# Martinsos/edlib

Hardware: AMD Instinct MI355X
Metric: GCUPS (cell updates/s), 1M x 150bp HW reads vs 5Mb target (higher is better)
Workload: dtype u32

## Files before the change

edlib_amd/csrc/engine.hip:

```cpp
#include "engine.hpp"
#include "flat_results.hpp"
#include <sched.h>

#if defined(__x86_64__)
#include <immintrin.h>
#endif
#include <algorithm>
#include <chrono>
#include <atomic>
#include <cmath>
#include <cstdarg>
#include <cstring>
#include <condition_variable>
#include <mutex>
#include <system_error>
#include <thread>

namespace edlib_amd {


static void build_eq8(std::vector<uint8_t>& eq8, const EdlibEqualityPair* eqs, int neq) {
    eq8.assign(256 * 256, 0);
    for (int a = 0; a < 256; ++a) eq8[a * 256 + a] = 1;
    for (int i = 0; i < neq; ++i) {
// ... 61 lines not shown
            if (tab.eq8.empty() ? (q == tab.idToByte[s]) : (tab.eq8[q * 256 + tab.idToByte[s]] != 0)) mask |= (uint16_t)(1u << s);
        tab.eqtbl[q] = mask;
    }
}


__global__ void __launch_bounds__(256)
alphabet_count_kernel(const uint8_t* __restrict__ qpool, const long long* __restrict__ qoff,
                      const uint8_t* __restrict__ tpool, const long long* __restrict__ toff,
                      int shared, const uint32_t* __restrict__ basePresence,
                      const int* __restrict__ unitIdx, int* __restrict__ out)
{
    __shared__ uint32_t s_seen[256];
    s_seen[threadIdx.x] = 0u;
    __syncthreads();
    const int u = unitIdx[blockIdx.x];
    auto scan = [&](const uint8_t* pool, long long lo, long long hi) {
        for (long long c = (lo >> 4) + threadIdx.x; (c << 4) < hi; c += 256) {
            const uint4 v = *reinterpret_cast<const uint4*>(pool + (c << 4));
            const uint32_t d[4] = {v.x, v.y, v.z, v.w};
            const long long at = c << 4;
            if (at >= lo && at + 16 <= hi) {
#pragma unroll
                for (int k = 0; k < 16; ++k) s_seen[(d[k >> 2] >> (8 * (k & 3))) & 0xffu] = 1u;
            } else {
#pragma unroll
                for (int k = 0; k < 16; ++k)
                    if (at + k >= lo && at + k < hi) s_seen[(d[k >> 2] >> (8 * (k & 3))) & 0xffu] = 1u;
            }
        }
    };
    scan(qpool, qoff[u], qoff[u + 1]);
    if (!shared) scan(tpool, toff[u], toff[u + 1]);
    __syncthreads();
    bool present = s_seen[threadIdx.x] != 0u;
    if (shared) present = present || ((basePresence[threadIdx.x >> 5] >> (threadIdx.x & 31)) & 1u);
    const int n = __syncthreads_count(present ? 1 : 0);
    if (threadIdx.x == 0) out[blockIdx.x] = n;
}

__global__ void __launch_bounds__(256)
alphabet_count_short_kernel(const uint8_t* __restrict__ qpool, const long long* __restrict__ qoff,
                            const uint8_t* __restrict__ tpool, const long long* __restrict__ toff,
                            int shared, const uint32_t* __restrict__ basePresence,
                            const int* __restrict__ unitIdx, int n, int* __restrict__ out)
{
    __shared__ uint32_t s_seen[4][64];
    const int lane = threadIdx.x & 63, wv = threadIdx.x >> 6;
    const int slot = blockIdx.x * 4 + wv;
    if (slot >= n) return;
    uint8_t* const seen = reinterpret_cast<uint8_t*>(s_seen[wv]);
    s_seen[wv][lane] = 0u;
    const int u = unitIdx[slot];
    auto scan = [&](const uint8_t* pool, long long lo, long long hi) {
        for (long long c = (lo >> 4) + lane; (c << 4) < hi; c += 64) {
            const uint4 v = *reinterpret_cast<const uint4*>(pool + (c << 4));
            const uint32_t d[4] = {v.x, v.y, v.z, v.w};
            const long long at = c << 4;
#pragma unroll
            for (int k = 0; k < 16; ++k)
                if (at + k >= lo && at + k < hi) seen[(d[k >> 2] >> (8 * (k & 3))) & 0xffu] = 1;
        }
    };
    scan(qpool, qoff[u], qoff[u + 1]);
    if (!shared) scan(tpool, toff[u], toff[u + 1]);
    __builtin_amdgcn_fence(__ATOMIC_RELEASE, "wavefront");
    __builtin_amdgcn_wave_barrier();
    uint32_t w = s_seen[wv][lane];
    if (shared) {
        const uint32_t bits = (basePresence[lane >> 3] >> (4 * (lane & 7))) & 0xfu;
        w |= (bits & 1u) | ((bits & 2u) << 7) | ((bits & 4u) << 14) | ((bits & 8u) << 21);
    }
    int cnt = ((w & 0xffu) != 0) + ((w & 0xff00u) != 0) + ((w & 0xff0000u) != 0) + ((w & 0xff000000u) != 0);
#pragma unroll
    for (int off = 32; off >= 1; off >>= 1) cnt += __shfl_xor(cnt, off, 64);
    if (lane == 0) out[slot] = cnt;
}


Batch::~Batch() {
    DeviceGuard guard(device_);
    if (side_) { (void)hipStreamSynchronize(side_); pool_stream_release(side_); }
    if (aux_) { (void)hipStreamSynchronize(aux_); (void)hipStreamDestroy(aux_); }
    if (stream_) { (void)hipStreamSynchronize(stream_); pool_stream_release(stream_); }
    wideGateRelease();
    for (auto& p : scanEvents_) { pool_event_release(p.first, device_); pool_event_release(p.second, device_); }
}

int roundup(int x, int q) { return (x + q - 1) / q * q; }

int Batch::init(const char* queries, const long long* qoff, int n, const char* targets,
                const long long* toff, int numTargets, EdlibAlignConfig cfg, int device, bool bothStrands, bool hits)
{
    if (n < 0 || (numTargets != 1 && numTargets != n)) { set_error("bad batch shape"); return 1; }
    if (hits) {
        if (numTargets != 1 || bothStrands) { set_error("hit-list read batch: one shared target, one strand"); return 1; }
        if (cfg.mode != EDLIB_MODE_HW) { set_error("hit-list read batch: config.mode must be EDLIB_MODE_HW (SHW and NW have no hit list)"); return 1; }
        if (cfg.task != EDLIB_TASK_DISTANCE) {
            set_error("hit-list read batch: config.task must be EDLIB_TASK_DISTANCE (start locations and paths: align the chosen windows with a pair batch)");
            return 1;
        }
        if (cfg.k < 0) { set_error("hit-list read batch: config.k must be >= 0 (got %d)", cfg.k); return 1; }
        for (int u = 0; u < n; ++u)
            if (qoff[u + 1] - qoff[u] > 32LL * kMaxReadWords) {
                set_error("hit-list read batch: read %d has %lld bases, the limit is %d", u, qoff[u + 1] - qoff[u], 32 * kMaxReadWords);
                return 1;
            }
        bool seen[256] = {false};
        int sigma = 0;
        for (long long j = toff[0]; j < toff[1]; ++j) if (!seen[(uint8_t)targets[j]]) { seen[(uint8_t)targets[j]] = true; ++sigma; }
        if (sigma > 16) { set_error("hit-list read batch: the target has %d distinct symbols, the limit is 16", sigma); return 1; }
    }
    hits_ = hits;
    if (bothStrands && (numTargets != 1 || n > 0x3fffffff)) { set_error("bad both-strand batch shape"); return 1; }
    if (check_device(device)) return 1;
    keep_config(cfg, cfg_, eqs_);
    device_ = device;
    strands_ = bothStrands;
    shared_ = (numTargets == 1);
    if (copy_offsets(qoff, n, "query", qoff_)) return 1;
    const int numReads = n;
    const long long qb = qoff[0];
    if (strands_) {
        n = 2 * numReads;
        qoff_.resize((size_t)n + 1);
        for (int i = 0; i < numReads; ++i) { qoff_[2 * i] = 2 * (qoff[i] - qb); qoff_[2 * i + 1] = 2 * (qoff[i] - qb) + (qoff[i + 1] - qoff[i]); }
        qoff_[n] = 2 * (qoff[numReads] - qb);
    }
    n_ = n;
    if (copy_offsets(toff, numTargets, "target", toff_)) return 1;
    const long long qbytes = qoff_[n] - qoff_[0], tbytes = toff_[numTargets] - toff_[0];
    build_tables(tab_, reinterpret_cast<const uint8_t*>(targets) + toff_[0], tbytes,
                 eqs_.data(), (int)eqs_.size());

    pool_quarantine(false);
    DeviceGuard guard(device_);
    EDLIB_AMD_HIP(guard.status);
    EDLIB_AMD_HIP(pool_stream(&stream_));
    EDLIB_AMD_HIP(evRun0_.create()); EDLIB_AMD_HIP(evRun1_.create());

    const long long tb = toff_[0];
    if (!strands_) for (auto& v : qoff_) v -= qb;
    for (auto& v : toff_) v -= tb;
    {
        const bool inlineT = qbytes + tbytes <= (1 << 20), inlineQ = inlineT && !strands_;
        size_t at = 0;
        auto take = [&](size_t bytes) { const size_t o = at; at = (at + bytes + 15) & ~(size_t)15; return o; };
        const size_t oQoff = take(qoff_.size() * sizeof(long long)), oToff = take(toff_.size() * sizeof(long long));
        const size_t oTlut = take(256), oId = take(256), oEq4 = take(512), oPres = take(32);
        const size_t oQ = inlineQ ? take((size_t)qbytes + 16) : 0, oT = inlineT ? take((size_t)tbytes + 16) : 0;
        EDLIB_AMD_HIP(d_in_.alloc(at));
        EDLIB_AMD_HIP(h_in_.alloc(at));
        uint8_t* h = h_in_.p;
        memcpy(h + oQoff, qoff_.data(), qoff_.size() * sizeof(long long));
        memcpy(h + oToff, toff_.data(), toff_.size() * sizeof(long long));
        memcpy(h + oTlut, tab_.tlut, 256); memcpy(h + oId, tab_.idToByte, 256);
        memcpy(h + oEq4, tab_.eqtbl, 512); memcpy(h + oPres, tab_.presence, 32);
        d_qoff_.alias(d_in_.p + oQoff, qoff_.size()); d_toff_.alias(d_in_.p + oToff, toff_.size());
        d_tlut_.alias(d_in_.p + oTlut, 256); d_idToByte_.alias(d_in_.p + oId, 256);
        d_eqtbl_.alias(d_in_.p + oEq4, 256); d_presence_.alias(d_in_.p + oPres, 8);
        if (inlineQ) {
            if (qbytes) memcpy(h + oQ, queries + qb, (size_t)qbytes);
            memset(h + oQ + qbytes, 0, 16);
            d_qpool_.alias(d_in_.p + oQ, (size_t)qbytes + 16);
        } else {
            EDLIB_AMD_HIP(d_qpool_.alloc((size_t)qbytes + 16));
// ... 868 lines not shown
```

edlib_amd/csrc/engine.hpp:

```cpp
#pragma once
#include "../../include/edlib_amd.h"
#include "common.hpp"
#include "pair_kernels.hpp"
#include "lanepair.hpp"
#include "reads_kernels.hpp"
#include "cross_kernels.hpp"
#include "window_kernels.hpp"
#include "strands.hpp"

#include <chrono>
#include <deque>
#include <functional>
#include <memory>
#include <vector>

namespace edlib_amd {

struct Tables {
    uint8_t tlut[256];
    uint8_t idToByte[256];
    int sigmaT = 0;
    uint32_t presence[8];
    uint16_t eqtbl[256];
    std::vector<uint8_t> eq8;
// ... 100 lines not shown
    int alphabetLength = 0;
    bool hasEnds = false, hasStarts = false, hasAlignment = false;
    LocList ends, starts;
    const uint8_t* opsView = nullptr;
    int opsViewLen = 0;
};

struct Lap;
struct ViewLayout;

class Batch {
public:
    virtual ~Batch();
    int init(const char* queries, const long long* qoff, int n,
             const char* targets, const long long* toff, int numTargets,
             EdlibAlignConfig cfg, int device, bool bothStrands = false,
             bool hits = false);
    int run();
    int runImpl();
    int results(EdlibAlignResult* out);
    int resultsFlat(int* status, int* editDistance, int* numLocations, int* alphabetLength, long long* locOffsets,
                    int** endLocations, int** startLocations, long long* alnOffsets, unsigned char** alignment);
    int resultsView(EdlibAmdResultsView* out);
    int cigarView(int format, const char** chars, const long long** offsets);
    int strandView(EdlibAmdStrandView* out);
    int hitsView(EdlibAmdReadHits* out);
    bool isHits() const { return hits_; }
    EdlibAmdBatchStats stats{};
    void finishStats();

private:
    EdlibAlignConfig cfg_{};
    std::vector<EdlibEqualityPair> eqs_;
    int device_ = 0;
    bool shared_ = false;
    int n_ = 0;
    std::vector<long long> qoff_, toff_;
    bool strands_ = false;
    PinBuf h_strand_;
    int outN() const { return strands_ ? n_ / 2 : n_; }
    int unitOf(int u) const { return strands_ ? 2 * u + h_strand_.p[u] : u; }
    void setStrand(int read, int code) { h_strand_.p[read] = (uint8_t)(code & kStrandReverse); h_strand_.p[outN() + read] = (code & kStrandBoth) ? 1 : 0; }
    int resolveStrandsOnHost(std::vector<UnitResult>& res);
    int hostStrandCounts_[4] = {0, 0, 0, 0};
    int strandCounts(int counts[4]);
    Tables tab_;
    hipStream_t stream_ = nullptr;
    Event evRun0_, evRun1_, evA_, evB_;

    DevBuf<uint8_t> d_in_;
    PinBuf h_in_;
    DevBuf<uint8_t> d_qpool_, d_tpool_, d_tlut_, d_idToByte_, d_eq8_;
    DevBuf<uint16_t> d_eqtbl_;
    hipError_t uploadEq8();
    DevBuf<uint32_t> d_presence_;
    DevBuf<long long> d_qoff_, d_toff_;

    std::vector<int> emptyUnits_, readUnits_, pairUnits_;
    std::vector<int> longUnits_;
    std::vector<int> pairNow_;
    int beginRun(hipError_t guardStatus);
    int enqueueWordSteps();
    int endRun();
    void resetRecords(std::vector<UnitResult>& res);
    void answerEmptyUnits(std::vector<UnitResult>& res);
    int runFlatPhase(std::vector<UnitResult>& res, Lap& lap);
    int runLongReads(std::vector<UnitResult>& res, Lap& lap);
    int runPairPhase(std::vector<UnitResult>& res, Lap& lap);
    int runStartsPhase(std::vector<UnitResult>& res, Lap& lap);
    int runPathsPhase(std::vector<UnitResult>& res, Lap& lap);
    void startStats();
    bool flatDone_ = false;

    struct ReadGroup {
        int nwords = 0, nslots = 0, numSegments = 1, segLen = 0, warm = 0, mMin = 0;
        std::vector<int> perm;
        DevBuf<int> d_perm, d_qlen, d_kinit, d_alphaExtra, d_segBest, d_segCnt, d_segPos;
        DevBuf<int> d_best, d_total, d_pos, d_flags;
        DevBuf<uint32_t> d_peq;
        bool zeroCopy = false; PinBuf hostOut;
        std::vector<int> ovfSlots; std::vector<long long> ovfOff; DevBuf<int> d_ovfPool;
        DevBuf<int> d_lvMap, d_lvBest, d_lvCnt, d_lvPos; std::vector<int> lvMap; int lvS = 0, lvCap = 0; bool lvValid = false;
        DevBuf<int> d_list;
        int nreal = -1;
        bool mates = false; DevBuf<int> d_win;
    };
    static constexpr int kLastLevelCap = 16;
    int listOpenSlots(ReadGroup& g, int kDone, std::vector<int>& out);
    DevBuf<uint8_t> d_selTmp_;
    std::vector<std::unique_ptr<ReadGroup>> groups_;
    DevBuf<uint32_t> d_tpk_, d_trows_;
    DevBuf<unsigned long long> d_wordSteps_;
    PinBuf h_wordSteps_; bool wordStepsPending_ = false;
    DevBuf<unsigned long long> d_ringSteps_; PinBuf h_ringSteps_; bool ringStepsUsed_ = false;
    unsigned long long* ringStepsCounter();
    bool banded_ = false;
    int syms_ = 4;
    int packTarget();
    int runReads();
    int makeGroup(const std::vector<int>& units, int words, std::unique_ptr<ReadGroup>& g, long long oneRoundWaves = 0);
    int runGroupScans(ReadGroup& g, bool fullOnly);
    int runGroupExact(ReadGroup& g);
    int collectGroup(ReadGroup& g, std::vector<UnitResult>& res);
    int seedThreshold(const ReadGroup& g, bool fullOnly) const;
    int buildSeedIndex();
    int runSeedPass(ReadGroup& g, int k);
    DevBuf<uint32_t> d_seedCnt_, d_seedOff_, d_seedPos_;
    DevBuf<uint8_t> d_seedTmp_;
    bool hits_ = false, hitsHaveRun_ = false, hitsFetched_ = false;
    long long hitCap_ = 0, numHits_ = 0;
    int hitSlots_ = 0;
    DevBuf<int> d_hitSlotUnit_;
    DevBuf<unsigned long long> d_hitCount_, d_hitKey_, d_hitSkey_;
    DevBuf<int> d_hitVal_, d_hitUnit_;
    DevBuf<uint32_t> d_hitIdx_, d_hitSidx_, d_hitHead_, d_hitAt_;
    DevBuf<long long> d_hitTotal_;
    DevBuf<uint8_t> d_hitTmp_, d_hitOut_;
    PinBuf h_hitCount_, h_hits_;
    std::vector<unsigned long long> hostHitKey_; std::vector<int> hostHitVal_;
    int growHitList(long long cap);
    int runReadHits();
    int scanGroupHits(ReadGroup& g, int slotBase);
    int hitsScanBanded(ReadGroup& g, int slotBase, const int* d_slotmap, int nlanes, int numSegments, int segLen, int warm);
    struct Piece { long long off; int len; int thr; };
    int scanPieces(const std::vector<Piece>& pieces, bool filter, std::vector<std::pair<int, int>>* cand,
                   std::vector<uint8_t>* overflow, std::vector<int>* best);
    int solveLongReads(std::vector<UnitResult>& res, std::vector<int>& fallback);
    bool filterScan_ = false;
    struct ChainArgs { const uint32_t* in = nullptr; uint32_t* out = nullptr; const int* src = nullptr; int inLanes = 0, blocks = 0; const int* rowBase = nullptr; };
    ChainArgs chain_;
    int solveTallFull(const std::vector<int>& units, std::vector<UnitResult>& res, std::vector<int>& handBack);
    int collectReads(std::vector<UnitResult>& res);
    bool readsCollected_ = true;
    int scanGroup(ReadGroup& g, int mode, const int* d_slotmap, int nlanes, int kcap, const int* d_kinit,
                  int numSegments, int segLen, int warm, int* segBest, int* segCnt, int* segPos, int cap,
                  const long long* posOff, const int* posCap, bool unbanded = false,
                  unsigned long long* wordSteps = nullptr, const uint32_t* peqDense = nullptr,
                  const int* qlenDense = nullptr, bool peqBottom = false);

    DevBuf<PairDesc> d_descs_;
    DevBuf<unsigned long long> d_peq64_;
    DevBuf<StoreEntry> d_store_;
    DevBuf<int> d_aux_, d_out3_, d_outScore_, d_outCount_, d_outLast_, d_posPool_, d_opsLen_, d_alpha_;
    DevBuf<uint8_t> d_ops_;
    DevBuf<long long> d_opsOff_;
    int solve(int mode, bool wantPositions, bool wantPath, const std::vector<UnitSpec>& units, SolveOut& out,
              int ring = 0, int ringH = 1);
    int solveChunk(int mode, bool wantPositions, bool wantPath, const std::vector<UnitSpec>& units,
                   size_t a, size_t b, SolveOut& out, int ring, int ringH);
    static const int kWide = -1;
    static const int kRing32 = -2;
    bool ring32_fits(const std::vector<UnitSpec>& units, size_t a, size_t b, int G) const;
    DevBuf<unsigned long long> d_wide_; DevBuf<unsigned> d_wabort_; PinBuf h_wabort_;
    int wideCap_ = -1;
    struct WidePlan { int slots = 1; size_t perLaunch = 1; };
    int planWide(int mode, PairDesc* descs, size_t n, WidePlan& plan);
    int launchWide(int mode, const PairScanArgs& a, const PairDesc* hostDescs, size_t n, const WidePlan& plan);
    int checkWide();
    bool wideSerial_ = false;
    bool wideGateHeld_ = false;
    void wideGateRelease();
    int solveWideSplit(const std::vector<UnitSpec>& units, std::vector<int>& out, int ring = 0);
    struct KnownSplit { long long qoff; int m; long long toff; int T; int score; int row, left, right; };
    std::vector<KnownSplit> knownSplits_;
    int solveGlobalDistances(const std::vector<UnitSpec>& units, std::vector<int>& score, std::vector<OpsOut>* paths = nullptr);
    int solveSemiGlobal(int mode, bool wantPositions, const std::vector<UnitSpec>& units, SolveOut& out);
    int solveSemiGlobalUnits(int mode, bool wantPositions, const std::vector<UnitSpec>& units, SolveOut& out);
    int solveBanded(const BandLadder& ladder, bool wantPositions, const std::vector<UnitSpec>& units, SolveOut& out);
    int alphabetLengthsBegin(hipEvent_t after = nullptr);
    bool alphaDeferred_ = false;
    int alphabetLengthsEnd(std::vector<UnitResult>& res);
    std::vector<int> alphaUnits_; bool alphaOnHost_ = false, alphaPending_ = false; long long alphaBytes_ = 0;
    hipStream_t side_ = nullptr;
    DevBuf<int> d_alphaIdx_, d_alphaOut_; PinBuf alphaPin_;
    struct PathPiece { long long qoff; int m; long long toff; int T; int score; };
    int hirschbergLevel(const std::vector<PathPiece>& big, std::vector<int>& splitRow,
                        std::vector<int>& leftScore, std::vector<int>& rightScore);
    int solvePaths(const std::vector<PathPiece>& jobs, std::vector<OpsOut>& opsOut, std::vector<int>& status);
    std::vector<std::shared_ptr<PinBuf>> opsKeep_;
    std::deque<std::vector<uint8_t>> opsOwned_;

    int qlen(int u) const { return (int)(qoff_[u + 1] - qoff_[u]); }
    long long tbase(int u) const { return shared_ ? toff_[0] : toff_[u]; }
    int tlen(int u) const { return shared_ ? (int)(toff_[1] - toff_[0]) : (int)(toff_[u + 1] - toff_[u]); }

    void scanTimerStart();
    void scanTimerStop();
    std::vector<std::pair<hipEvent_t, hipEvent_t>> scanEvents_;
    size_t scanEventsUsed_ = 0;

    std::vector<UnitResult> results_, work_;
    std::vector<UnitSpec> startUnits_; std::vector<std::pair<int, int>> startWhere_; std::vector<int> live_;
    bool haveResults_ = false;
    long long algoBase_ = -1;
    bool algoDirty_ = false;
    std::vector<int> pairSpecsFor_;
    std::vector<UnitSpec> pairSpecs_, selScratch_; std::vector<size_t> whoScratch_; std::vector<int> lvlScratch_, scoreMain_;
    SolveOut soMain_, soLevel_;
    int pairSpecsVersion_ = 0, levelSpecsVersion_ = -1, shapeVersion_ = -1, alphaIsPairsVersion_ = -1;
    bool alphaIsPairs_ = false;
    struct PairShape { size_t minBlocks = 0, maxBlocks = 0; int minLenLo = 0, minLenHi = 0, maxDiff = 0; } shape_;
    long long levelPeqWords_ = 0;
    bool levelAllReady_ = false;
    PinBuf h_levelSpecs_, h_levelScore_;
    DevBuf<LevelSpec> d_levelSpecs_;
    DevBuf<PairDesc> d_descsAll_;
    DevBuf<unsigned long long> d_peqAll_;
    hipStream_t aux_ = nullptr;
    Event evLevelIn_, evLevelPeq_;
    int prepareLevelAll(const std::vector<UnitSpec>& units);
    std::function<void()> whileScanning_;
    int runLevelAll(const std::vector<UnitSpec>& units, int ring, int ringH, int ringBlocks, int cap, int kcap, int nbMax);
    int laneSpecsVersion_ = -1;
    long long lanePlaneWords_ = -1, laneTgtWords_ = 0;
    bool laneReady_ = false;
    PinBuf h_laneUnits_, h_laneScore_;
    DevBuf<lanepair::LaneUnit> d_laneUnits_;
    DevBuf<lanepair::Plane2> d_lanePlanes_;
    DevBuf<lanepair::Tgt2> d_laneTgts_;
    DevBuf<int> d_laneFlags_, d_laneScore_;
    Event evLanePack_;
// ... 89 lines not shown
```

edlib_amd/csrc/engine_reads.hip:

```cpp
#include "engine.hpp"

#include <algorithm>
#include <chrono>
#include <cmath>
#include <condition_variable>
#include <cstring>
#include <mutex>
#include <thread>

namespace edlib_amd {

__global__ void __launch_bounds__(256)
seed_thresholds_kernel(int* __restrict__ kinit, const int* __restrict__ best, const int* __restrict__ cnt, int n)
{
    const int i = blockIdx.x * blockDim.x + threadIdx.x;
    if (i < n && cnt[i] > 0 && best[i] < kinit[i]) kinit[i] = best[i];
}


int Batch::scanGroup(ReadGroup& g, int mode, const int* d_slotmap, int nlanes, int kcap, const int* d_kinit,
                     int numSegments, int segLen, int warm, int* segBest, int* segCnt, int* segPos, int cap,
                     const long long* posOff, const int* posCap, bool unbanded, unsigned long long* wordSteps,
                     const uint32_t* peqDense, const int* qlenDense, bool peqBottom)
{
    ReadScanArgs a{};
    a.peq = peqDense ? peqDense : g.d_peq.p; a.tpk = d_tpk_.p; a.trows = d_trows_.p; a.targetLength = tlen(0);
    if (mode == EDLIB_MODE_SHW) a.targetLength = (int)std::min<long long>(a.targetLength, 64LL * g.nwords + 1);
    a.qlen = qlenDense ? qlenDense : g.d_qlen.p; a.kinit = d_kinit; a.slotmap = d_slotmap; a.nlanes = nlanes;
    a.numSegments = numSegments; a.segLen = segLen; a.warm = warm;
    a.segBest = segBest; a.segCnt = segCnt; a.segPos = segPos; a.cap = cap;
    a.posOff = posOff; a.posCap = posCap;
    a.kcap = kcap; a.wordSteps = wordSteps ? wordSteps : d_wordSteps_.p;
    a.filter = filterScan_ ? 1 : 0;
    a.bottomAligned = peqBottom ? 1 : 0;
    a.chainIn = chain_.in; a.chainOut = chain_.out; a.chainSrc = chain_.src; a.chainInLanes = chain_.inLanes;
    a.chainBlocks = chain_.blocks; a.rowBase = chain_.rowBase;
    const bool chained = chain_.in != nullptr || chain_.out != nullptr;
    static const bool dbg = getenv("EDLIB_AMD_DEBUG") != nullptr;
    if (dbg) {
        EDLIB_AMD_HIP(hipStreamSynchronize(stream_));
        fprintf(stderr, "[edlib_amd] scanGroup nwords=%d mode=%d nlanes=%d S=%d segLen=%d warm=%d cap=%d kcap=%d slotmap=%p posOff=%p\n",
                g.nwords, mode, nlanes, numSegments, segLen, warm, cap, kcap, (const void*)d_slotmap, (const void*)posOff);
    }
    scanTimerStart();
    const bool longGroup = g.nwords > kMaxReadWords;
    const long long colsScanned = std::min<long long>(a.targetLength, (long long)numSegments * segLen) + (long long)(numSegments - 1) * warm;
    const bool fullHeight = banded_ && mode == EDLIB_MODE_HW && unbanded && (chained || syms_ > 4 || longGroup);
    const bool bandedKernel = !fullHeight && banded_ && mode == EDLIB_MODE_HW && (!unbanded || syms_ > 4 || longGroup);
    if (peqBottom && (fullHeight || bandedKernel)) EDLIB_AMD_HIP(hipErrorInvalidValue);
    if (fullHeight) {
        EDLIB_AMD_HIP(launch_scan_reads_full(g.nwords, syms_, a, stream_));
        stats.word_steps += (long long)((nlanes + 63) / 64 * 64) * g.nwords * colsScanned;
    } else if (bandedKernel) EDLIB_AMD_HIP(launch_scan_reads_banded(g.nwords, syms_, a, stream_));
    else {
        EDLIB_AMD_HIP(launch_scan_reads(g.nwords, mode, a, stream_));
        stats.word_steps += (long long)((nlanes + 63) / 64 * 64) * g.nwords * colsScanned;
    }
    scanTimerStop();
    if (dbg) {
        EDLIB_AMD_HIP(hipStreamSynchronize(stream_));
        fprintf(stderr, "[edlib_amd] scanGroup done\n");
    }
    return 0;
}

void plan_segments(int nlanes, int T, int mode, int warmFull, long long wantWaves,
                          int& S, int& segLen, int& warm, int minSegCols)
{
    S = 1; segLen = roundup(T, 16); warm = 0;
    if (mode != EDLIB_MODE_HW) return;
    const long long nrblk = ((long long)nlanes + 63) / 64;
    long long want = (wantWaves + nrblk - 1) / nrblk;
    want = std::max(1LL, std::min<long long>(want, std::min(65535, std::max(1, T / minSegCols))));
    if (warmFull > 0) want = std::max(1LL, std::min<long long>(want, std::max<long long>(1, T / (4LL * warmFull))));
    segLen = roundup((int)((T + want - 1) / want), 16);
    S = (T + segLen - 1) / segLen;
    warm = warmFull;
}

int Batch::runReads()
{
    if (groups_.empty()) return 0;
    stats.path |= 1;
    bool seed = false;
    for (auto& gp : groups_) seed = seed || seedThreshold(*gp, false) >= 0;
    if (seed && buildSeedIndex()) return 1;
    for (auto& gp : groups_) if (runGroupScans(*gp, false)) return 1;
    const int mode = (cfg_.mode == EDLIB_MODE_HW || cfg_.mode == EDLIB_MODE_SHW) ? (int)cfg_.mode : (int)EDLIB_MODE_NW;
    for (auto& gp : groups_)
        if (gp->mates) EDLIB_AMD_HIP(launch_resolve_strands(gp->d_perm.p, gp->d_best.p, gp->d_total.p, gp->nslots, mode, cfg_.k,
                                                            gp->d_win.p, stream_));
    for (auto& gp : groups_) if (runGroupExact(*gp)) return 1;
    return 0;
}

int Batch::runGroupScans(ReadGroup& g, bool fullOnly)
{
    const int T = tlen(0);
    const int mode = (cfg_.mode == EDLIB_MODE_HW || cfg_.mode == EDLIB_MODE_SHW) ? (int)cfg_.mode : (int)EDLIB_MODE_NW;
    const bool banded = banded_ && mode == EDLIB_MODE_HW;
    const int kNoCap = 0x3fffffff;
    static const bool dbgLadder = getenv("EDLIB_AMD_DEBUG") != nullptr;
    EDLIB_AMD_HIP(launch_build_peq_reads(g.nwords, syms_, d_qpool_.p, d_qoff_.p, g.d_perm.p, g.nslots,
                                         d_eqtbl_.p, d_presence_.p, cfg_.k, g.d_peq.p, g.d_qlen.p,
                                         g.d_kinit.p, g.d_alphaExtra.p, stream_));
    const int kSeed = seedThreshold(g, fullOnly);
    const int kFirstMax = kSeed >= 0 ? kSeed : std::max(8, g.nwords / 2);
    int kFirst = (kSeed >= 0 && cfg_.k >= 0) ? std::min(kSeed, cfg_.k) : kFirstMax;
    bool twoPass = !fullOnly && banded && (cfg_.k < 0 || cfg_.k > kFirst) && 32 * g.nwords > kFirst;
    std::vector<int> ladder;
    g.lvValid = false;
    auto probe_scan = [&](const std::vector<int>& map, int kc, std::vector<int>& bestOut) -> int {
        const int nm = (int)map.size();
        int S2, segLen2, warm2;
        plan_segments(nm, T, mode, g.warm, 16384, S2, segLen2, warm2);
        const size_t items = (size_t)nm * S2;
        DevBuf<int> d_map, d_sb, d_sc;
        EDLIB_AMD_HIP(d_map.alloc(nm)); EDLIB_AMD_HIP(d_sb.alloc(items)); EDLIB_AMD_HIP(d_sc.alloc(items));
        EDLIB_AMD_HIP(hipMemcpyAsync(d_map.p, map.data(), nm * sizeof(int), hipMemcpyHostToDevice, stream_));
        if (scanGroup(g, mode, d_map.p, nm, kc, g.d_kinit.p, S2, segLen2, warm2,
                      d_sb.p, d_sc.p, d_sb.p , 0, nullptr, nullptr)) return 1;
        std::vector<int> cnts(items), bests(items);
        EDLIB_AMD_HIP(hipMemcpyAsync(cnts.data(), d_sc.p, items * sizeof(int), hipMemcpyDeviceToHost, stream_));
        EDLIB_AMD_HIP(hipMemcpyAsync(bests.data(), d_sb.p, items * sizeof(int), hipMemcpyDeviceToHost, stream_));
        EDLIB_AMD_HIP(hipStreamSynchronize(stream_));
        bestOut.assign(nm, -1);
        for (int i = 0; i < nm; ++i) {
            int b = 0x7fffffff;
            for (int sg = 0; sg < S2; ++sg)
                if (cnts[(size_t)i * S2 + sg] > 0) b = std::min(b, bests[(size_t)i * S2 + sg]);
            if (b <= kc) bestOut[i] = b;
        }
        return 0;
    };
    auto price_ladder = [&](const std::vector<int>& sample, size_t nOpen, int nReal) -> int {
        const int kTop = std::min(64, 32 * g.nwords - 1);
        std::vector<int> obest;
        if (probe_scan(sample, kTop, obest)) return 1;
        static const int cand[6] = {12, 16, 24, 32, 48, 64};
        auto words = [&](int t) { return std::min<double>(g.nwords, 1.0 + std::max(0, t - 6) / 8.0); };
        auto frac_le = [&](int t) {
// ... 7 lines not shown
            for (int q = 0; q < 6; ++q) {
                if (!((mask >> q) & 1)) continue;
                if (cand[q] <= kFirst || cand[q] > kTop) { ok = false; break; }
                cost += reach * words(cand[q]);
                reach = 1.0 - frac_le(cand[q]);
            }
            if (!ok) continue;
            cost += reach * g.nwords;
            if (cost < bestCost - 1e-9) { bestCost = cost; bestMask = mask; }
        }
        for (int q = 0; q < 6; ++q) if ((bestMask >> q) & 1) ladder.push_back(cand[q]);
        if (dbgLadder) {
            fprintf(stderr, "[edlib_amd] ladder nwords=%d kFirst=%d open=%zu/%d levels:", g.nwords, kFirst, nOpen, nReal);
            for (int t : ladder) fprintf(stderr, " %d(%.2f)", t, frac_le(t));
            fprintf(stderr, " full\n");
        }
        return 0;
    };
    if (twoPass && g.nslots >= 16384 && kSeed < 0) {
        const int np = std::max(512, std::min(2048, g.nslots / 32));
        std::vector<int> probe(np);
        for (int i = 0; i < np; ++i) probe[i] = (int)((long long)i * g.nslots / np);
        std::vector<int> pbest;
        if (probe_scan(probe, kFirst, pbest)) return 1;
        int resolved = 0, real = 0;
        std::vector<int> hist(kFirstMax + 1, 0);
        std::vector<int> open;
        for (int i = 0; i < np; ++i) {
            if (g.perm[probe[i]] < 0) continue;
            ++real;
            if (pbest[i] >= 0) { ++resolved; ++hist[pbest[i]]; }
            else if (i == 0 || probe[i] != probe[i - 1]) open.push_back(probe[i]);
        }
        if (resolved > 0) {
            int acc = 0, kq = kFirstMax;
            for (int d = 0; d <= kFirstMax; ++d) { acc += hist[d]; if (acc * 1000LL >= resolved * 995LL) { kq = d; break; } }
            kFirst = std::max(4, std::min(kFirstMax, kq));
        }
        if (real > 0 && resolved * 10 < real * 3) twoPass = false;
        if (twoPass && (int)open.size() * 10 > real && open.size() >= 32 && price_ladder(open, open.size(), real)) return 1;
    }
    std::vector<int> todo;
    bool haveTodo = false;
    if (kSeed >= 0) {
        if (runSeedPass(g, kFirst)) return 1;
        if (twoPass) {
            if (listOpenSlots(g, kFirst, todo)) return 1;
            haveTodo = true;
            if (g.nreal < 0) { g.nreal = 0; for (int u : g.perm) g.nreal += u >= 0; }
            if (g.nslots >= 16384 && todo.size() * 10 > (size_t)g.nreal && todo.size() >= 32) {
                const size_t nsm = std::min<size_t>(2048, todo.size());
                std::vector<int> sample(nsm);
                for (size_t i = 0; i < nsm; ++i) sample[i] = todo[i * todo.size() / nsm];
                if (price_ladder(sample, todo.size(), g.nreal)) return 1;
            }
        }
    } else {
        if (scanGroup(g, mode, nullptr, g.nslots, twoPass ? kFirst : kNoCap, g.d_kinit.p, g.numSegments, g.segLen,
                      g.warm, g.d_segBest.p, g.d_segCnt.p, g.d_segPos.p, 8, nullptr, nullptr, fullOnly)) return 1;
        const bool chained = chain_.in != nullptr || chain_.out != nullptr;
        EDLIB_AMD_HIP(launch_merge_segments(g.d_segBest.p, g.d_segCnt.p, g.d_segPos.p, g.numSegments, 8,
                                            g.nslots, nullptr, 16, g.d_best.p, g.d_total.p, g.d_pos.p,
                                            g.d_flags.p, stream_, chained ? kOvfRescan : kOvfGatherGroup));
    }
    ladder.push_back(kNoCap);
    int kDone = kFirst;
    for (size_t lv = 0; twoPass && lv < ladder.size(); ++lv) {
        const int kcapL = ladder[lv];
        const bool last = kcapL == kNoCap;
        if (!haveTodo && listOpenSlots(g, kDone, todo)) return 1;
        haveTodo = false;
        if (todo.empty()) break;
        {
            const size_t no = todo.size();
            int S2, segLen2, warm2;
            plan_segments((int)no, T, mode, g.warm, 65536, S2, segLen2, warm2);
            const size_t items = no * (size_t)S2;
            const int capL = last ? kLastLevelCap : 8;
            EDLIB_AMD_HIP(g.d_lvMap.ensure(no)); EDLIB_AMD_HIP(g.d_lvBest.ensure(items)); EDLIB_AMD_HIP(g.d_lvCnt.ensure(items));
            EDLIB_AMD_HIP(g.d_lvPos.ensure(items * capL));
            int *d_map = g.d_lvMap.p, *d_sb = g.d_lvBest.p, *d_sc = g.d_lvCnt.p, *d_sp = g.d_lvPos.p;
            EDLIB_AMD_HIP(hipMemcpyAsync(d_map, todo.data(), no * sizeof(int), hipMemcpyHostToDevice, stream_));
            bool plain = false;
            if (last && no >= 4096) {
                const int np2 = 64;
                std::vector<int> sub(np2);
                for (int i = 0; i < np2; ++i) sub[i] = todo[(size_t)((long long)i * no / np2)];
                int S3, segLen3, warm3;
                plan_segments(np2, T, mode, g.warm, 16384, S3, segLen3, warm3);
                const size_t it3 = (size_t)np2 * S3;
                DevBuf<int> d_m3, d_b3, d_c3, d_p3; DevBuf<unsigned long long> d_ws;
                EDLIB_AMD_HIP(d_m3.alloc(np2)); EDLIB_AMD_HIP(d_b3.alloc(it3)); EDLIB_AMD_HIP(d_c3.alloc(it3));
                EDLIB_AMD_HIP(d_p3.alloc(it3 * 8)); EDLIB_AMD_HIP(d_ws.alloc(1));
                EDLIB_AMD_HIP(hipMemcpyAsync(d_m3.p, sub.data(), np2 * sizeof(int), hipMemcpyHostToDevice, stream_));
                EDLIB_AMD_HIP(hipMemsetAsync(d_ws.p, 0, sizeof(unsigned long long), stream_));
                if (scanGroup(g, mode, d_m3.p, np2, kNoCap, g.d_kinit.p, S3, segLen3, warm3,
                              d_b3.p, d_c3.p, d_p3.p, 8, nullptr, nullptr, false, d_ws.p)) return 1;
                unsigned long long ws = 0;
                EDLIB_AMD_HIP(hipMemcpyAsync(&ws, d_ws.p, sizeof ws, hipMemcpyDeviceToHost, stream_));
                EDLIB_AMD_HIP(hipStreamSynchronize(stream_));
                const double cols = (double)np2 * ((double)T + (double)(S3 - 1) * warm3);
                plain = (double)ws >= 0.85 * g.nwords * cols;
                stats.word_steps += (long long)ws;
            }
            const bool bottom = plain && mode == EDLIB_MODE_HW && syms_ == 4 && g.nwords <= kMaxReadWords &&
                                chain_.in == nullptr && chain_.out == nullptr;
            const size_t no64 = (no + 63) / 64 * 64;
            std::vector<int> perm2(no64, -1);
            for (size_t i = 0; i < no; ++i) perm2[i] = g.perm[todo[i]];
            DevBuf<int> d_perm2, d_qlen2, d_kinit2, d_extra2; DevBuf<uint32_t> d_peq2;
            EDLIB_AMD_HIP(d_perm2.alloc(no64)); EDLIB_AMD_HIP(d_qlen2.alloc(no64)); EDLIB_AMD_HIP(d_kinit2.alloc(no64));
            EDLIB_AMD_HIP(d_extra2.alloc(no64)); EDLIB_AMD_HIP(d_peq2.alloc(no64 * (size_t)syms_ * g.nwords));
            EDLIB_AMD_HIP(hipMemcpyAsync(d_perm2.p, perm2.data(), no64 * sizeof(int), hipMemcpyHostToDevice, stream_));
            EDLIB_AMD_HIP(launch_build_peq_reads(g.nwords, syms_, d_qpool_.p, d_qoff_.p, d_perm2.p, (int)no64,
                                                 d_eqtbl_.p, d_presence_.p, cfg_.k, d_peq2.p, d_qlen2.p,
                                                 d_kinit2.p, d_extra2.p, stream_, bottom));
            const int seedCols = 4096;
            DevBuf<int> d_b0, d_c0, d_p0;
            if (mode == EDLIB_MODE_HW && last && no >= 4096 && S2 > 1 && T >= 16 * seedCols) {
                EDLIB_AMD_HIP(d_b0.alloc(no)); EDLIB_AMD_HIP(d_c0.alloc(no)); EDLIB_AMD_HIP(d_p0.alloc(no * 8));
                if (scanGroup(g, mode, nullptr, (int)no, kcapL, d_kinit2.p, 1, seedCols, 0,
                              d_b0.p, d_c0.p, d_p0.p, 8, nullptr, nullptr, plain, nullptr, d_peq2.p, d_qlen2.p, bottom)) return 1;
                hipLaunchKernelGGL(seed_thresholds_kernel, dim3((unsigned)((no + 255) / 256)), dim3(256), 0, stream_,
                                   d_kinit2.p, d_b0.p, d_c0.p, (int)no);
                EDLIB_AMD_HIP(hipGetLastError());
            }
            if (scanGroup(g, mode, nullptr, (int)no, kcapL, d_kinit2.p, S2, segLen2, warm2,
                          d_sb, d_sc, d_sp, capL, nullptr, nullptr, plain, nullptr, d_peq2.p, d_qlen2.p, bottom)) return 1;
            EDLIB_AMD_HIP(launch_merge_segments(d_sb, d_sc, d_sp, S2, capL, (int)no, d_map, 16,
                                                g.d_best.p, g.d_total.p, g.d_pos.p, g.d_flags.p, stream_,
                                                last ? kOvfGatherLevel : kOvfRescan));
            EDLIB_AMD_HIP(hipStreamSynchronize(stream_));
            if (last) { g.lvValid = true; g.lvS = S2; g.lvCap = capL; g.lvMap.swap(todo); }
            if (dbgLadder) fprintf(stderr, "[edlib_amd] level kcap=%d: %zu slots rescanned (plain=%d)\n", kcapL, no, (int)plain);
        }
        kDone = kcapL;
    }
    return 0;
}

int Batch::listOpenSlots(ReadGroup& g, int kDone, std::vector<int>& out)
{
    size_t tmp = 0;
    EDLIB_AMD_HIP(select_slots_scratch_bytes(g.nslots, &tmp));
    EDLIB_AMD_HIP(d_selTmp_.ensure(tmp));
    EDLIB_AMD_HIP(g.d_list.ensure((size_t)g.nslots + 1));
    int* count = g.d_list.p + g.nslots;
    EDLIB_AMD_HIP(launch_select_open_slots(g.d_perm.p, g.d_total.p, g.d_qlen.p, cfg_.k, kDone, g.nslots, g.d_list.p, count,
                                           d_selTmp_.p, d_selTmp_.bytes(), stream_, g.mates));
    int n = 0;
    EDLIB_AMD_HIP(hipMemcpyAsync(&n, count, sizeof(int), hipMemcpyDeviceToHost, stream_));
    EDLIB_AMD_HIP(hipStreamSynchronize(stream_));
    out.resize((size_t)n);
    if (n > 0) {
        EDLIB_AMD_HIP(hipMemcpyAsync(out.data(), g.d_list.p, (size_t)n * sizeof(int), hipMemcpyDeviceToHost, stream_));
        EDLIB_AMD_HIP(hipStreamSynchronize(stream_));
    }
    return 0;
}


int Batch::seedThreshold(const ReadGroup& g, bool fullOnly) const
{
    const long long T = tlen(0);
    if (fullOnly || !banded_ || cfg_.mode != EDLIB_MODE_HW || syms_ != 4 || cfg_.additionalEqualitiesLength > 0 ||
        g.nwords > kMaxReadWords || chain_.in != nullptr || chain_.out != nullptr)
        return -1;
    if (T < 64LL * 32 * g.nwords || g.nslots < 1024 || (long long)g.nslots * T < (1LL << 30)) return -1;
    int kf = -1;
    for (int k = 16; k >= 0 && kf < 0; --k) {
        const int L = g.mMin / (k + 1);
        if (L >= kSeedQ && (double)(k + 1) * (double)T <= std::ldexp(1.0, 2 * L) / 8.0) kf = k;
    }
    return (kf >= 0 && kf >= std::min(8, cfg_.k >= 0 ? cfg_.k : 8)) ? kf : -1;
}

int Batch::buildSeedIndex()
{
    const int T = tlen(0);
    EDLIB_AMD_HIP(d_seedCnt_.ensure((size_t)kSeedBuckets + 1));
    EDLIB_AMD_HIP(d_seedOff_.ensure((size_t)kSeedBuckets + 1));
    EDLIB_AMD_HIP(d_seedPos_.ensure((size_t)T));
    size_t tmp = 0;
    EDLIB_AMD_HIP(seed_index_scratch_bytes(&tmp));
    EDLIB_AMD_HIP(d_seedTmp_.ensure(tmp));
    scanTimerStart();
    EDLIB_AMD_HIP(launch_build_seed_index(d_tpk_.p, T, d_seedCnt_.p, d_seedOff_.p, d_seedPos_.p, d_seedTmp_.p,
                                          d_seedTmp_.bytes(), stream_));
    scanTimerStop();
    return 0;
}

int Batch::runSeedPass(ReadGroup& g, int k)
{
    const int T = tlen(0);
    DevBuf<int> d_back;
    EDLIB_AMD_HIP(d_back.alloc((size_t)g.nslots + 1));
    int* backCount = d_back.p + g.nslots;
    EDLIB_AMD_HIP(hipMemsetAsync(backCount, 0, sizeof(int), stream_));
    SeedArgs a{};
    a.peq = g.d_peq.p; a.qlen = g.d_qlen.p; a.perm = g.d_perm.p; a.tpk = d_tpk_.p; a.targetLength = T;
    a.seedOff = d_seedOff_.p; a.seedPos = d_seedPos_.p; a.nslots = g.nslots; a.k = k;
    a.best = g.d_best.p; a.total = g.d_total.p; a.pos = g.d_pos.p; a.flags = g.d_flags.p;
    a.backSlots = d_back.p; a.backCount = backCount; a.wordSteps = d_wordSteps_.p;
    scanTimerStart();
    EDLIB_AMD_HIP(launch_seed_verify(g.nwords, a, stream_));
    scanTimerStop();
    int nb = 0;
    EDLIB_AMD_HIP(hipMemcpyAsync(&nb, backCount, sizeof(int), hipMemcpyDeviceToHost, stream_));
// ... 376 lines not shown
```

Measured before the change: 3.164 million.

## Run census scan on side stream while speculatively preparing plain-kernel rescan

The 64-read census scan that decides whether the last ladder level can use the plain kernel now runs on a separate stream. Meanwhile the main stream speculatively builds the peq tables and pre-scan seeds assuming the plain path, and redoes that preparation if the census says otherwise. The lane-to-unit permutation is now built on the device instead of on the host, and the census and pre-scan buffers are kept on the group for reuse rather than reallocated each time. The cost is an extra stream and event, and the whole preparation is wasted when the speculation is wrong.

Result: no change. 3.175 million, median of 6 (+0.3%).

```diff
diff --git a/edlib_amd/csrc/engine.hip b/edlib_amd/csrc/engine.hip
--- a/edlib_amd/csrc/engine.hip
+++ b/edlib_amd/csrc/engine.hip
@@ -167,6 +167,7 @@
     DeviceGuard guard(device_);
     if (side_) { (void)hipStreamSynchronize(side_); pool_stream_release(side_); }
     if (aux_) { (void)hipStreamSynchronize(aux_); (void)hipStreamDestroy(aux_); }
+    if (census_) { (void)hipStreamSynchronize(census_); pool_stream_release(census_); }
     if (stream_) { (void)hipStreamSynchronize(stream_); pool_stream_release(stream_); }
     wideGateRelease();
     for (auto& p : scanEvents_) { pool_event_release(p.first, device_); pool_event_release(p.second, device_); }
diff --git a/edlib_amd/csrc/engine.hpp b/edlib_amd/csrc/engine.hpp
--- a/edlib_amd/csrc/engine.hpp
+++ b/edlib_amd/csrc/engine.hpp
@@ -206,10 +206,14 @@
         std::vector<int> ovfSlots; std::vector<long long> ovfOff; DevBuf<int> d_ovfPool;
         DevBuf<int> d_lvMap, d_lvBest, d_lvCnt, d_lvPos; std::vector<int> lvMap; int lvS = 0, lvCap = 0; bool lvValid = false;
         DevBuf<int> d_list;
+        DevBuf<int> d_cnMap, d_cnBest, d_cnCnt, d_cnPos, d_psBest, d_psCnt, d_psPos;
+        DevBuf<unsigned long long> d_cnSteps; PinBuf h_cnSteps;
         int nreal = -1;
         bool mates = false; DevBuf<int> d_win;
     };
     static constexpr int kLastLevelCap = 16;
+    static constexpr int kPreScanCols = 4096;
+    hipStream_t census_ = nullptr; Event evCensus_;
     int listOpenSlots(ReadGroup& g, int kDone, std::vector<int>& out);
     DevBuf<uint8_t> d_selTmp_;
     std::vector<std::unique_ptr<ReadGroup>> groups_;
@@ -260,7 +264,7 @@
                   int numSegments, int segLen, int warm, int* segBest, int* segCnt, int* segPos, int cap,
                   const long long* posOff, const int* posCap, bool unbanded = false,
                   unsigned long long* wordSteps = nullptr, const uint32_t* peqDense = nullptr,
-                  const int* qlenDense = nullptr, bool peqBottom = false);
+                  const int* qlenDense = nullptr, bool peqBottom = false, hipStream_t on = nullptr);
 
     DevBuf<PairDesc> d_descs_;
     DevBuf<unsigned long long> d_peq64_;
diff --git a/edlib_amd/csrc/engine_reads.hip b/edlib_amd/csrc/engine_reads.hip
--- a/edlib_amd/csrc/engine_reads.hip
+++ b/edlib_amd/csrc/engine_reads.hip
@@ -17,12 +17,20 @@
     if (i < n && cnt[i] > 0 && best[i] < kinit[i]) kinit[i] = best[i];
 }
 
+__global__ void __launch_bounds__(256)
+lane_units_kernel(int* __restrict__ out, const int* __restrict__ perm, const int* __restrict__ map, int n, int n64)
+{
+    const int i = blockIdx.x * blockDim.x + threadIdx.x;
+    if (i < n64) out[i] = i < n ? perm[map[i]] : -1;
+}
+
 
 int Batch::scanGroup(ReadGroup& g, int mode, const int* d_slotmap, int nlanes, int kcap, const int* d_kinit,
                      int numSegments, int segLen, int warm, int* segBest, int* segCnt, int* segPos, int cap,
                      const long long* posOff, const int* posCap, bool unbanded, unsigned long long* wordSteps,
-                     const uint32_t* peqDense, const int* qlenDense, bool peqBottom)
-{
+                     const uint32_t* peqDense, const int* qlenDense, bool peqBottom, hipStream_t on)
+{
+    const hipStream_t st = on ? on : stream_;
     ReadScanArgs a{};
     a.peq = peqDense ? peqDense : g.d_peq.p; a.tpk = d_tpk_.p; a.trows = d_trows_.p; a.targetLength = tlen(0);
     if (mode == EDLIB_MODE_SHW) a.targetLength = (int)std::min<long long>(a.targetLength, 64LL * g.nwords + 1);
@@ -42,21 +50,21 @@
         fprintf(stderr, "[edlib_amd] scanGroup nwords=%d mode=%d nlanes=%d S=%d segLen=%d warm=%d cap=%d kcap=%d slotmap=%p posOff=%p\n",
                 g.nwords, mode, nlanes, numSegments, segLen, warm, cap, kcap, (const void*)d_slotmap, (const void*)posOff);
     }
-    scanTimerStart();
+    if (st == stream_) scanTimerStart();
     const bool longGroup = g.nwords > kMaxReadWords;
     const long long colsScanned = std::min<long long>(a.targetLength, (long long)numSegments * segLen) + (long long)(numSegments - 1) * warm;
     const bool fullHeight = banded_ && mode == EDLIB_MODE_HW && unbanded && (chained || syms_ > 4 || longGroup);
     const bool bandedKernel = !fullHeight && banded_ && mode == EDLIB_MODE_HW && (!unbanded || syms_ > 4 || longGroup);
     if (peqBottom && (fullHeight || bandedKernel)) EDLIB_AMD_HIP(hipErrorInvalidValue);
     if (fullHeight) {
-        EDLIB_AMD_HIP(launch_scan_reads_full(g.nwords, syms_, a, stream_));
+        EDLIB_AMD_HIP(launch_scan_reads_full(g.nwords, syms_, a, st));
         stats.word_steps += (long long)((nlanes + 63) / 64 * 64) * g.nwords * colsScanned;
-    } else if (bandedKernel) EDLIB_AMD_HIP(launch_scan_reads_banded(g.nwords, syms_, a, stream_));
+    } else if (bandedKernel) EDLIB_AMD_HIP(launch_scan_reads_banded(g.nwords, syms_, a, st));
     else {
-        EDLIB_AMD_HIP(launch_scan_reads(g.nwords, mode, a, stream_));
+        EDLIB_AMD_HIP(launch_scan_reads(g.nwords, mode, a, st));
         stats.word_steps += (long long)((nlanes + 63) / 64 * 64) * g.nwords * colsScanned;
     }
-    scanTimerStop();
+    if (st == stream_) scanTimerStop(); else ++stats.scan_launches;
     if (dbg) {
         EDLIB_AMD_HIP(hipStreamSynchronize(stream_));
         fprintf(stderr, "[edlib_amd] scanGroup done\n");
@@ -230,49 +238,80 @@
             int *d_map = g.d_lvMap.p, *d_sb = g.d_lvBest.p, *d_sc = g.d_lvCnt.p, *d_sp = g.d_lvPos.p;
             EDLIB_AMD_HIP(hipMemcpyAsync(d_map, todo.data(), no * sizeof(int), hipMemcpyHostToDevice, stream_));
             bool plain = false;
-            if (last && no >= 4096) {
-                const int np2 = 64;
-                std::vector<int> sub(np2);
+            const bool census = last && no >= 4096;
+            const bool plainOk = mode == EDLIB_MODE_HW && syms_ == 4 && g.nwords <= kMaxReadWords &&
+                                 chain_.in == nullptr && chain_.out == nullptr;
+            const bool speculate = census && plainOk;
+            const int np2 = 64;
+            std::vector<int> sub;
+            int S3 = 1, segLen3 = 0, warm3 = 0;
+            unsigned long long* h_ws = nullptr;
+            if (census) {
+                if (!g.h_cnSteps.p) EDLIB_AMD_HIP(g.h_cnSteps.alloc(sizeof(unsigned long long)));
+                h_ws = reinterpret_cast<unsigned long long*>(g.h_cnSteps.p);
+                sub.resize(np2);
                 for (int i = 0; i < np2; ++i) sub[i] = todo[(size_t)((long long)i * no / np2)];
-                int S3, segLen3, warm3;
                 plan_segments(np2, T, mode, g.warm, 16384, S3, segLen3, warm3);
                 const size_t it3 = (size_t)np2 * S3;
-                DevBuf<int> d_m3, d_b3, d_c3, d_p3; DevBuf<unsigned long long> d_ws;
-                EDLIB_AMD_HIP(d_m3.alloc(np2)); EDLIB_AMD_HIP(d_b3.alloc(it3)); EDLIB_AMD_HIP(d_c3.alloc(it3));
-                EDLIB_AMD_HIP(d_p3.alloc(it3 * 8)); EDLIB_AMD_HIP(d_ws.alloc(1));
-                EDLIB_AMD_HIP(hipMemcpyAsync(d_m3.p, sub.data(), np2 * sizeof(int), hipMemcpyHostToDevice, stream_));
-                EDLIB_AMD_HIP(hipMemsetAsync(d_ws.p, 0, sizeof(unsigned long long), stream_));
-                if (scanGroup(g, mode, d_m3.p, np2, kNoCap, g.d_kinit.p, S3, segLen3, warm3,
-                              d_b3.p, d_c3.p, d_p3.p, 8, nullptr, nullptr, false, d_ws.p)) return 1;
-                unsigned long long ws = 0;
-                EDLIB_AMD_HIP(hipMemcpyAsync(&ws, d_ws.p, sizeof ws, hipMemcpyDeviceToHost, stream_));
-                EDLIB_AMD_HIP(hipStreamSynchronize(stream_));
+                EDLIB_AMD_HIP(g.d_cnMap.ensure(np2)); EDLIB_AMD_HIP(g.d_cnBest.ensure(it3)); EDLIB_AMD_HIP(g.d_cnCnt.ensure(it3));
+                EDLIB_AMD_HIP(g.d_cnPos.ensure(it3 * 8)); EDLIB_AMD_HIP(g.d_cnSteps.ensure(1));
+                if (speculate) {
+                    if (!census_) EDLIB_AMD_HIP(pool_stream(&census_));
+                    EDLIB_AMD_HIP(evCensus_.create());
+                    EDLIB_AMD_HIP(hipEventRecord(evCensus_.e, stream_));
+                    EDLIB_AMD_HIP(hipStreamWaitEvent(census_, evCensus_.e, 0));
+                }
+            }
+            auto issue_census = [&]() -> int {
+                const hipStream_t cs = speculate ? census_ : stream_;
+                EDLIB_AMD_HIP(hipMemcpyAsync(g.d_cnMap.p, sub.data(), np2 * sizeof(int), hipMemcpyHostToDevice, cs));
+                EDLIB_AMD_HIP(hipMemsetAsync(g.d_cnSteps.p, 0, sizeof(unsigned long long), cs));
+                if (scanGroup(g, mode, g.d_cnMap.p, np2, kNoCap, g.d_kinit.p, S3, segLen3, warm3, g.d_cnBest.p, g.d_cnCnt.p,
+                              g.d_cnPos.p, 8, nullptr, nullptr, false, g.d_cnSteps.p, nullptr, nullptr, false, cs)) return 1;
+                EDLIB_AMD_HIP(hipMemcpyAsync(h_ws, g.d_cnSteps.p, sizeof *h_ws, hipMemcpyDeviceToHost, cs));
+                return 0;
+            };
+            auto census_answer = [&]() -> int {
+                EDLIB_AMD_HIP(hipStreamSynchronize(speculate ? census_ : stream_));
                 const double cols = (double)np2 * ((double)T + (double)(S3 - 1) * warm3);
-                plain = (double)ws >= 0.85 * g.nwords * cols;
-                stats.word_steps += (long long)ws;
-            }
-            const bool bottom = plain && mode == EDLIB_MODE_HW && syms_ == 4 && g.nwords <= kMaxReadWords &&
-                                chain_.in == nullptr && chain_.out == nullptr;
+                plain = (double)*h_ws >= 0.85 * g.nwords * cols;
+                stats.word_steps += (long long)*h_ws;
+                return 0;
+            };
+            if (census && !speculate && (issue_census() || census_answer())) return 1;
             const size_t no64 = (no + 63) / 64 * 64;
-            std::vector<int> perm2(no64, -1);
-            for (size_t i = 0; i < no; ++i) perm2[i] = g.perm[todo[i]];
             DevBuf<int> d_perm2, d_qlen2, d_kinit2, d_extra2; DevBuf<uint32_t> d_peq2;
             EDLIB_AMD_HIP(d_perm2.alloc(no64)); EDLIB_AMD_HIP(d_qlen2.alloc(no64)); EDLIB_AMD_HIP(d_kinit2.alloc(no64));
             EDLIB_AMD_HIP(d_extra2.alloc(no64)); EDLIB_AMD_HIP(d_peq2.alloc(no64 * (size_t)syms_ * g.nwords));
-            EDLIB_AMD_HIP(hipMemcpyAsync(d_perm2.p, perm2.data(), no64 * sizeof(int), hipMemcpyHostToDevice, stream_));
-            EDLIB_AMD_HIP(launch_build_peq_reads(g.nwords, syms_, d_qpool_.p, d_qoff_.p, d_perm2.p, (int)no64,
-                                                 d_eqtbl_.p, d_presence_.p, cfg_.k, d_peq2.p, d_qlen2.p,
-                                                 d_kinit2.p, d_extra2.p, stream_, bottom));
-            const int seedCols = 4096;
-            DevBuf<int> d_b0, d_c0, d_p0;
-            if (mode == EDLIB_MODE_HW && last && no >= 4096 && S2 > 1 && T >= 16 * seedCols) {
-                EDLIB_AMD_HIP(d_b0.alloc(no)); EDLIB_AMD_HIP(d_c0.alloc(no)); EDLIB_AMD_HIP(d_p0.alloc(no * 8));
-                if (scanGroup(g, mode, nullptr, (int)no, kcapL, d_kinit2.p, 1, seedCols, 0,
-                              d_b0.p, d_c0.p, d_p0.p, 8, nullptr, nullptr, plain, nullptr, d_peq2.p, d_qlen2.p, bottom)) return 1;
+            hipLaunchKernelGGL(lane_units_kernel, dim3((unsigned)((no64 + 255) / 256)), dim3(256), 0, stream_,
+                               d_perm2.p, g.d_perm.p, d_map, (int)no, (int)no64);
+            EDLIB_AMD_HIP(hipGetLastError());
+            const bool prime = mode == EDLIB_MODE_HW && census && S2 > 1 && T >= 16 * kPreScanCols;
+            auto prepare = [&](bool plainK) -> int {
+                const bool bottomK = plainK && plainOk;
+                EDLIB_AMD_HIP(launch_build_peq_reads(g.nwords, syms_, d_qpool_.p, d_qoff_.p, d_perm2.p, (int)no64,
+                                                     d_eqtbl_.p, d_presence_.p, cfg_.k, d_peq2.p, d_qlen2.p,
+                                                     d_kinit2.p, d_extra2.p, stream_, bottomK));
+                if (!prime) return 0;
+                EDLIB_AMD_HIP(g.d_psBest.ensure(no)); EDLIB_AMD_HIP(g.d_psCnt.ensure(no)); EDLIB_AMD_HIP(g.d_psPos.ensure(no * 8));
+                if (scanGroup(g, mode, nullptr, (int)no, kcapL, d_kinit2.p, 1, kPreScanCols, 0, g.d_psBest.p, g.d_psCnt.p,
+                              g.d_psPos.p, 8, nullptr, nullptr, plainK, nullptr, d_peq2.p, d_qlen2.p, bottomK)) return 1;
                 hipLaunchKernelGGL(seed_thresholds_kernel, dim3((unsigned)((no + 255) / 256)), dim3(256), 0, stream_,
-                                   d_kinit2.p, d_b0.p, d_c0.p, (int)no);
+                                   d_kinit2.p, g.d_psBest.p, g.d_psCnt.p, (int)no);
                 EDLIB_AMD_HIP(hipGetLastError());
-            }
+                return 0;
+            };
+            if (speculate) {
+                const auto steps0 = stats.word_steps; const auto launches0 = stats.scan_launches;
+                const size_t events0 = scanEventsUsed_;
+                if (prepare(true)) return 1;
+                if (issue_census() || census_answer()) return 1;
+                if (!plain) {
+                    stats.word_steps = steps0 + (long long)*h_ws; stats.scan_launches = launches0 + 1; scanEventsUsed_ = events0;
+                    if (prepare(false)) return 1;
+                }
+            } else if (prepare(plain)) return 1;
+            const bool bottom = plain && plainOk;
             if (scanGroup(g, mode, nullptr, (int)no, kcapL, d_kinit2.p, S2, segLen2, warm2,
                           d_sb, d_sc, d_sp, capL, nullptr, nullptr, plain, nullptr, d_peq2.p, d_qlen2.p, bottom)) return 1;
             EDLIB_AMD_HIP(launch_merge_segments(d_sb, d_sc, d_sp, S2, capL, (int)no, d_map, 16,
```
